# mic-rud/Learned-Compression-of-Point-Cloud-Geometry-and-Attributes

Hardware: AMD Instinct MI355X
Metric: encode+decode Mpoints/sec (higher is better)
Workload: dtype f32

## Files before the change

### include/pcc_hip.h

```cpp
#ifndef PCC_HIP_H
#define PCC_HIP_H

#include <stdint.h>

#ifdef __cplusplus
extern "C" {
#endif

#define PCC_OK 0
#define PCC_ERR_ARG (-1)
#define PCC_ERR_HIP (-2)
#define PCC_ERR_UNSUPPORTED (-3)
#define PCC_ERR_DATA (-4)

#define PCC_ACT_NONE 0
#define PCC_ACT_RELU 1
#define PCC_ACT_LEAKY_RELU 2

int pcc_version(void);
const char* pcc_last_error(void);
int pcc_device_count(void);
int pcc_device_name(int dev, char* out, int out_len);

int64_t pcc_hash_capacity(int64_t n);
// ... 24 lines not shown

int32_t pcc_color_jitter_chunk(void);
int64_t pcc_color_jitter_scratch_bytes(int64_t n, int32_t nbatch);
int pcc_color_jitter(const float* rgb, int64_t n, const int64_t* offsets, int32_t nbatch, const float* params,
                     const int32_t* order, float* out, void* scratch, int64_t scratch_bytes, void* stream);

int pcc_voxelize(const float* xyz, const int32_t* batch, int64_t n, int32_t nbatch, const float* attr, int32_t c,
                 float origin_x, float origin_y, float origin_z, float voxel, int32_t rounding, uint64_t* keys,
                 int32_t* vals, int64_t cap, int32_t* scratch, int32_t* out_coords, int32_t* out_first,
                 int32_t* out_npts, int64_t* out_sum, int32_t* out_row, int64_t* out_count, void* stream);

int pcc_kernel_map(const int32_t* out_coords, int64_t n_out, const uint64_t* in_keys,
                   const int32_t* in_vals, int64_t in_cap, int32_t ksize, int32_t step,
                   int32_t sign, int32_t* nbr, uint32_t* row_mask, int64_t* pair_count,
                   void* stream);

int pcc_pair_count(const uint32_t* row_mask, int64_t n_out, int64_t* pair_count, void* stream);

int64_t pcc_order_scratch_bytes(int64_t n);
int pcc_order_rows_by_mask(const uint32_t* row_mask, const int32_t* coords, int64_t n,
                           int32_t block_log2, int32_t tensor_stride, int32_t* order, uint32_t* group_mask32,
                           void* scratch, int64_t scratch_bytes, void* stream);
int pcc_permute_map_rows(const int32_t* nbr, const int32_t* order, int64_t n, int32_t K, int32_t* nbr_sorted, void* stream);

int64_t pcc_small_map_max(void);
int32_t pcc_small_paths(int32_t mask);
int pcc_small_kernel_map(const int32_t* out_coords, int64_t n_out, const uint64_t* in_keys, const int32_t* in_vals, int64_t in_cap,
                         int32_t ksize, int32_t step, int32_t sign, int32_t* nbr, uint32_t* row_mask, int32_t* order,
                         uint32_t* group_mask32, void* scratch, int64_t scratch_bytes, void* stream);

// ... 21 lines not shown
int pcc_epilogue_bwd(const float* dout, const float* c, const float* film, int64_t n, int32_t channels, int32_t act,
                     float* dc, float* dfilm, void* stream);

int64_t pcc_cast_colsum_scratch_elems(int32_t channels);
int pcc_cast_colsum(const float* x, int64_t n, int32_t channels, uint16_t* out_bf16, float* colsum, float* scratch,
                    int64_t scratch_elems, void* stream);

int64_t pcc_conv_packed_elems_x3(int32_t K, int32_t cin, int32_t cout);
int pcc_conv_pack_weights_x3(const float* w, int32_t K, int32_t cin, int32_t cout, uint16_t* w_packed, void* stream);
int pcc_conv_fwd_x3(const float* fin, int64_t n_in, int32_t cin, const uint16_t* w_packed, const float* bias,
                    const int32_t* nbr, const int32_t* order, const uint32_t* group_mask32, int32_t K, float* fout,
                    int64_t n_out, int32_t cout, int32_t act, const float* film, const float* residual, void* stream);

int pcc_im2col_thin(const float* fin, int32_t cin, const int32_t* nbr, int64_t n_out, int32_t K, float* out, int32_t k2,
                    void* stream);

int pcc_gather_sum_fwd(const float* scores, int32_t ld, const int32_t* nbr, int32_t K, int32_t cout,
                       const float* bias, float* out, int64_t n_out, int32_t act, void* stream);

int pcc_gather_rows(const float* src, int32_t c, const int32_t* idx, int64_t n, float* out,
                    int32_t accumulate, void* stream);

int pcc_scatter_rows(const float* src, int32_t c, const int32_t* idx, int64_t n, float* out,
                     void* stream);
int pcc_scatter_add_rows(const float* src, int32_t c, const int32_t* idx, int64_t n, float* out,
                         void* stream);

int pcc_compact_rows(const uint8_t* mask, int64_t n, const int32_t* coords, int32_t* out_coords,
                     const float* feats, int32_t c, float* out_feats, int32_t* new_index,
                     int32_t* scratch, int64_t* out_count, void* stream);
// ... 109 lines not shown
```

### learned-compression-of-point-cloud-geometry-and-attributes_amd/_lib.py

```python
import ctypes
import os
import subprocess

_HERE = os.path.dirname(os.path.abspath(__file__))
SO_PATH = os.path.join(_HERE, "libpcc_hip.so")
_lib = None

c_void_p, c_int, c_i32, c_i64 = ctypes.c_void_p, ctypes.c_int, ctypes.c_int32, ctypes.c_int64

SIGNATURES = {
    "pcc_version": (c_int, []),
    "pcc_last_error": (ctypes.c_char_p, []),
    "pcc_device_count": (c_int, []),
    "pcc_device_name": (c_int, [c_int, ctypes.c_char_p, c_int]),
    "pcc_hash_capacity": (c_i64, [c_i64]),
    "pcc_hash_build": (c_int, [c_void_p, c_i64, c_void_p, c_void_p, c_i64, c_i32, c_void_p, c_void_p]),
    "pcc_hash_lookup": (c_int, [c_void_p, c_void_p, c_i64, c_i32, c_void_p, c_i64, c_void_p, c_void_p]),
    "pcc_scan_scratch_elems": (c_i64, [c_i64]),
    "pcc_stride_map": (c_int, [c_void_p, c_i64, c_i32, c_void_p, c_void_p, c_i64, c_void_p, c_void_p, c_void_p, c_void_p]),
    "pcc_children": (c_int, [c_void_p, c_i64, c_i32, c_i32, c_void_p, c_void_p, c_i64, c_void_p, c_void_p, c_void_p, c_void_p]),
    "pcc_augment_rotate": (c_int, [c_void_p, c_i64, c_void_p, c_i32, ctypes.c_float, c_void_p, c_void_p, c_i64, c_void_p, c_void_p, c_void_p,
                                   c_void_p, c_void_p]),
    "pcc_color_jitter_chunk": (c_i32, []),
    "pcc_color_jitter_scratch_bytes": (c_i64, [c_i64, c_i32]),
    "pcc_color_jitter": (c_int, [c_void_p, c_i64, c_void_p, c_i32, c_void_p, c_void_p, c_void_p, c_void_p, c_i64, c_void_p]),
    "pcc_voxelize": (c_int, [c_void_p, c_void_p, c_i64, c_i32, c_void_p, c_i32, ctypes.c_float, ctypes.c_float, ctypes.c_float, ctypes.c_float,
                             c_i32, c_void_p, c_void_p, c_i64, c_void_p, c_void_p, c_void_p, c_void_p, c_void_p, c_void_p, c_void_p,
                             c_void_p]),
    "pcc_kernel_map": (c_int, [c_void_p, c_i64, c_void_p, c_void_p, c_i64, c_i32, c_i32, c_i32, c_void_p, c_void_p, c_void_p, c_void_p]),
    "pcc_pair_count": (c_int, [c_void_p, c_i64, c_void_p, c_void_p]),
    "pcc_conv_packed_elems": (c_i64, [c_i32, c_i32, c_i32]),
    "pcc_conv_pack_weights": (c_int, [c_void_p, c_i32, c_i32, c_i32, c_void_p, c_void_p]),
    "pcc_order_scratch_bytes": (c_i64, [c_i64]),
    "pcc_order_rows_by_mask": (c_int, [c_void_p, c_void_p, c_i64, c_i32, c_i32, c_void_p, c_void_p, c_void_p, c_i64, c_void_p]),
    "pcc_permute_map_rows": (c_int, [c_void_p, c_void_p, c_i64, c_i32, c_void_p, c_void_p]),
    "pcc_conv_fwd": (c_int, [c_void_p, c_i64, c_i32, c_void_p, c_void_p, c_void_p, c_void_p, c_void_p, c_void_p, c_i32,
                             c_void_p, c_i64, c_i32, c_i32, c_void_p, c_void_p, c_void_p]),
    "pcc_conv_small_max": (c_i64, [c_i64]),
    "pcc_conv_kernel_name": (c_int, [c_i32, c_i64, c_i32, c_i32, c_i64, c_i32, c_i32, ctypes.c_char_p, c_i32]),
    "pcc_small_map_max": (c_i64, []),
    "pcc_small_paths": (c_i32, [c_i32]),
    "pcc_small_kernel_map": (c_int, [c_void_p, c_i64, c_void_p, c_void_p, c_i64, c_i32, c_i32, c_i32, c_void_p, c_void_p, c_void_p,
                                     c_void_p, c_void_p, c_i64, c_void_p]),
    "pcc_conv_packed_elems_bf16": (c_i64, [c_i32, c_i32, c_i32]),
    "pcc_conv_pack_weights_bf16": (c_int, [c_void_p, c_i32, c_i32, c_i32, c_void_p, c_void_p]),
    "pcc_conv_fwd_bf16": (c_int, [c_void_p, c_i64, c_i32, c_void_p, c_void_p, c_void_p, c_void_p, c_void_p, c_i32, c_void_p, c_i64,
                                  c_i32, c_i32, c_void_p, c_void_p, c_void_p]),
    "pcc_conv_packed_elems_x3": (c_i64, [c_i32, c_i32, c_i32]),
    "pcc_conv_pack_weights_x3": (c_int, [c_void_p, c_i32, c_i32, c_i32, c_void_p, c_void_p]),
    "pcc_conv_fwd_x3": (c_int, [c_void_p, c_i64, c_i32, c_void_p, c_void_p, c_void_p, c_void_p, c_void_p, c_i32, c_void_p, c_i64,
                                c_i32, c_i32, c_void_p, c_void_p, c_void_p]),
    "pcc_epilogue_fwd": (c_int, [c_void_p, c_void_p, c_void_p, c_i64, c_i32, c_i32, c_void_p, c_void_p]),
    "pcc_cast_colsum_scratch_elems": (c_i64, [c_i32]),
    "pcc_cast_colsum": (c_int, [c_void_p, c_i64, c_i32, c_void_p, c_void_p, c_void_p, c_i64, c_void_p]),
    "pcc_epilogue_bwd": (c_int, [c_void_p, c_void_p, c_void_p, c_i64, c_i32, c_i32, c_void_p, c_void_p, c_void_p]),
    "pcc_im2col_thin": (c_int, [c_void_p, c_i32, c_void_p, c_i64, c_i32, c_void_p, c_i32, c_void_p]),
    "pcc_gather_sum_fwd": (c_int, [c_void_p, c_i32, c_void_p, c_i32, c_i32, c_void_p, c_void_p, c_i64, c_i32, c_void_p]),
    "pcc_gather_rows": (c_int, [c_void_p, c_i32, c_void_p, c_i64, c_void_p, c_i32, c_void_p]),
    "pcc_scatter_rows": (c_int, [c_void_p, c_i32, c_void_p, c_i64, c_void_p, c_void_p]),
    "pcc_scatter_add_rows": (c_int, [c_void_p, c_i32, c_void_p, c_i64, c_void_p, c_void_p]),
    "pcc_compact_rows": (c_int, [c_void_p, c_i64, c_void_p, c_void_p, c_void_p, c_i32, c_void_p, c_void_p, c_void_p, c_void_p, c_void_p]),
    "pcc_topk_state_elems": (c_i64, [c_i32]),
    "pcc_topk_mask": (c_int, [c_void_p, c_i32, c_void_p, c_i64, c_i32, c_void_p, c_void_p, c_void_p, c_void_p]),
    "pcc_count_per_batch": (c_int, [c_void_p, c_i64, c_i32, c_void_p, c_void_p]),
    "pcc_sort_scratch_bytes": (c_i64, [c_i64]),
    "pcc_sort_coords": (c_int, [c_void_p, c_i64, c_void_p, c_void_p, c_i64, c_void_p]),
    "pcc_kernel_map_transpose": (c_int, [c_void_p, c_i64, c_i32, c_i64, c_void_p, c_void_p, c_void_p]),
    "pcc_conv_wgrad_scratch_elems": (c_i64, [c_i32, c_i32, c_i32]),
    "pcc_conv_wgrad_kernel_name": (c_int, [c_i32, c_i32, c_i32, c_i32, c_i64, ctypes.c_char_p, c_i32, c_void_p, c_void_p]),
    "pcc_conv_wgrad": (c_int, [c_void_p, c_i64, c_i32, c_void_p, c_i64, c_i32, c_void_p, c_void_p, c_void_p, c_i32, c_void_p, c_void_p,
                               c_i64, c_void_p]),
    "pcc_conv_wgrad_bf16": (c_int, [c_void_p, c_i64, c_i32, c_void_p, c_i64, c_i32, c_void_p, c_void_p, c_void_p, c_i32, c_void_p, c_void_p,
# ... 40 lines not shown
def build(force=False):
    args = ["make", "-s", "-C", os.path.join(_HERE, "csrc"), "-j4"]
    if force:
        subprocess.check_call(args + ["clean"])
    subprocess.check_call(args)
    check_kernel_resources()
    check_kernel_resources(os.path.join(_HERE, "build", "rans_lanes.resources.txt"), LANE_KERNELS)
    check_kernel_resources(os.path.join(_HERE, "build", "chconv.resources.txt"), CHCONV_KERNELS)
    check_kernel_resources(os.path.join(_HERE, "build", "augment.resources.txt"), AUGMENT_KERNELS)
    check_kernel_resources(os.path.join(_HERE, "build", "normals.resources.txt"), NORMALS_KERNELS)
    check_kernel_resources(os.path.join(_HERE, "build", "voxelize.resources.txt"), VOXELIZE_KERNELS)
    check_small_kernel_lds_reads()
    return SO_PATH


NO_SCRATCH_KERNELS = ("conv_small_kernel", "conv_mfma_buf_kernel", "conv_mfma_kernel")
LANE_KERNELS = ("rans_lanes_encode_kernel", "rans_lanes_pack_kernel", "rans_lanes_decode_kernel")
CHCONV_KERNELS = ("chconv_kernel",)
AUGMENT_KERNELS = ("jitter_partial_kernel", "jitter_mean_kernel", "jitter_apply_kernel", "rotate_clear_kernel", "rotate_insert_kernel",
                   "rotate_flag_kernel", "rotate_finalize_kernel")

NORMALS_KERNELS = ("estimate_normals_kernel",)
VOXELIZE_KERNELS = ("voxelize_clear_kernel", "voxelize_insert_kernel", "voxelize_flag_kernel", "voxelize_finalize_kernel",
                    "voxelize_accumulate_kernel")


def check_small_kernel_lds_reads(obj=None):
    import glob
    import re
    import shutil
    objdump = "/opt/rocm/lib/llvm/bin/llvm-objdump"
# ... 141 lines not shown
```

### learned-compression-of-point-cloud-geometry-and-attributes_amd/blocks.py

```python
import os

import torch
import torch.nn as nn

from . import _threads
from . import sparse as sp
from .sparse import (ACT_NONE, ACT_RELU, ConvChain, CoordMap, MinkowskiConvolution,
                     MinkowskiGenerativeConvolutionTranspose, MinkowskiPruning, MinkowskiReLU, SparseTensor)


class _NonNegativeParametrizer(nn.Module):
    def __init__(self, minimum=0.0, reparam_offset=2 ** -18):
        super().__init__()
        pedestal = float(reparam_offset) ** 2
        self.register_buffer("pedestal", torch.tensor([pedestal]))
        self.lower_bound = _Bound((float(minimum) + pedestal) ** 0.5)


class _Bound(nn.Module):
    def __init__(self, bound):
        super().__init__()
        self.register_buffer("bound", torch.tensor([float(bound)]))


# ... 52 lines not shown
            with torch.cuda.stream(side):
                job(side)
        except BaseException as e:
            for h in handoffs:
                h.fail(e)
            raise

    if x_map.n >= PREFETCH_THREAD_MIN_ROWS:
        x_map._cache[("prefetch_job",)] = st.job_thread("pcc-map-prefetch", dev).submit(run)
    else:
        run()
    x_map._cache[done_key] = True
    return True


PREFETCH_THREAD_MIN_ROWS = 8192


def prefetch_up_maps(x_map):
    first = _threads.Handoff()

    def job(side):
        cand = x_map.up(3)
        x_map.mfma_kernel_map(cand, 3, True)
        first.set(side.record_event())
        cand.mfma_kernel_map(cand, 3)
        cand.kernel_map(cand, 3)
        x_map._cache[("prefetch_event",)] = side.record_event()

    if _start_prefetch(x_map, ("okmap_prefetched",), job, [first]):
# ... 81 lines not shown
            self.occ_predict = ConvChain(_conv(N_out, N_out), MinkowskiReLU(), _conv(N_out, N_out))

    def forward(self, x, coords=None, k=None, full_predictions=False):
        if not self.predict:
            return self._follow(x, coords)
        in_map = x.map
        _join_prefetch_first(in_map)
        x = self.conv(x)
        _join_prefetch(in_map)
        if self.dense and self.condition_ablation is None:
            x = self.conv_2(x)
        pred = self.occ_predict(x, last_out_channels=None if full_predictions else 1)
        nb = x.map._nbatch if x.map._nbatch is not None else x.map.nbatch
        mask = sp.topk_mask(pred.F, pred.C, k, nb)
        kept = min(max(int(k[0]), 0), x.map.n) if nb == 1 and len(k) == 1 and not torch.is_grad_enabled() else None
        coords_kept, feats_kept, _, _ = sp.compact_rows(mask, x.C, x.F, expected=kept)
        up_map = CoordMap(coords_kept, x.map.stride, nbatch=x.map._nbatch)
        x = SparseTensor(feats_kept, coordinate_map=up_map)
        if not self.dense and self.condition_ablation is None:
            x = self.conv_2(x)
        return x, pred, up_map

    def _follow(self, Q, up_map):
        if not isinstance(up_map, CoordMap):
            up_map = CoordMap(sp._as_int_coords(up_map), Q.map.stride // 2, nbatch=Q.map._nbatch)
        return self.conv(Q, out_map=up_map)


class ConditionEncoder(nn.Module):

    def __init__(self, C_in, N_scales, N_features, condition_ablation=None):
        super().__init__()
# ... 42 lines not shown
```

### learned-compression-of-point-cloud-geometry-and-attributes_amd/csrc/conv.hip

```cpp
#include <stdlib.h>

#include <type_traits>

#include "common.h"

namespace pcc {

typedef float f32x2 __attribute__((ext_vector_type(2)));
typedef float f32x4 __attribute__((ext_vector_type(4)));
typedef float f32x16 __attribute__((ext_vector_type(16)));
typedef __bf16 bf16x8 __attribute__((ext_vector_type(8)));

struct ConvArgs {
    const float* fin;
    const float* w;
    const float* wp;
    const float* bias;
    const int32_t* nbr;
    const int32_t* order;
    const uint32_t* gmask;
    float* fout;
    const float* film;
    const float* residual;
    int64_t n_in, n_out;
    int cin, cout, coutp, K, act;
    int bf16;
};

__device__ __forceinline__ float apply_act(float v, int act) {
    if (act == PCC_ACT_RELU) return v > 0.0f ? v : 0.0f;
    if (act == PCC_ACT_LEAKY_RELU) return v > 0.0f ? v : 0.01f * v;
    return v;
}

__global__ __launch_bounds__(256) void pack_weights_kernel(const float* __restrict__ w, int K, int cin, int cout,
                                                           int cinp, int coutp, float* __restrict__ wp) {
    const int64_t total = (int64_t)K * cinp * coutp;
    for (int64_t e = (int64_t)blockIdx.x * blockDim.x + threadIdx.x; e < total; e += (int64_t)gridDim.x * blockDim.x) {
        const int s = (int)(e & 3);
        int64_t t = e >> 2;
        const int col = (int)(t % coutp);
// ... 597 lines not shown
        }
    }

#pragma unroll
    for (int m = 0; m < MT; ++m) {
#pragma unroll
        for (int n = 0; n < NT; ++n) {
#pragma unroll
            for (int reg = 0; reg < 16; ++reg) {
                const int col = nt * BN + wcol + 32 * n + r;
                if (col >= a.cout) continue;
                const float bcol = a.bias ? a.bias[col] : 0.0f;
                const int64_t pos = row0 + wrow + 32 * m + (reg & 3) + 8 * (reg >> 2) + 4 * h;
                if (pos >= a.n_out) continue;
                const int64_t row = a.order ? a.order[pos] : pos;
                float v = acc[m][n][reg] + bcol;
                if (a.film) {
                    const float* fr = a.film + row * (2 * (int64_t)a.cout);
                    v = v * fr[col] + fr[a.cout + col];
                }
                v = apply_act(v, a.act);
                if (a.residual) v += a.residual[row * a.cout + col];
                a.fout[row * a.cout + col] = v;
            }
        }
    }
#endif
}

template <int SC, int NS>
// ... 492 lines not shown
static int launch_thin_cin(const ConvPlan& p, const ConvArgs& a, hipStream_t st) {
    switch (a.cin) {
        case 1: return launch_thin<1>(p, a, st);
        case 2: return launch_thin<2>(p, a, st);
        case 3: return launch_thin<3>(p, a, st);
        case 4: return launch_thin<4>(p, a, st);
        case 6: return launch_thin<6>(p, a, st);
        case 8: return launch_thin<8>(p, a, st);
        case 12: return launch_thin<12>(p, a, st);
        case 16: return launch_thin<16>(p, a, st);
        case 24: return launch_thin<24>(p, a, st);
        default: return PCC_ERR_UNSUPPORTED;
    }
}

static int conv_fwd(ConvMode mode, const ConvArgs& a, void* stream) {
    const char* who = CONV_ENTRY[mode];
    int rc = check_shape(a, mode, who);
    if (rc != PCC_OK) return rc;
    PCC_REQUIRE(a.act >= 0 && a.act <= 2, "%s: bad activation %d", who, a.act);
    if (mode == CONV_F32 && a.n_out <= 0) return PCC_OK;
    if (mode != CONV_F32 || a.cin % 32 == 0) {
        PCC_REQUIRE(a.wp != nullptr, "%s: MFMA path (cin=%d) needs packed weights", who, a.cin);
        PCC_REQUIRE(((reinterpret_cast<uintptr_t>(a.fin) | reinterpret_cast<uintptr_t>(a.wp)) & 15) == 0,
                    "%s: fin and w_packed must be 16-byte aligned (16-byte LDS-DMA loads)", who);
    } else {
        PCC_REQUIRE(a.w != nullptr, "%s: thin path (cin=%d) needs raw weights", who, a.cin);
    }
    if (a.n_out <= 0) return PCC_OK;
    ConvPlan p;
// ... 70 lines not shown
                    int32_t act, const float* film, const float* residual, void* stream) {
    return conv_fwd(CONV_X3, {fin, nullptr, reinterpret_cast<const float*>(w_packed), bias, nbr, order, group_mask32, fout, film,
                              residual, n_in, n_out, cin, cout, round_up32(cout), K, act, 0}, stream);
}

int pcc_im2col_thin(const float* fin, int32_t cin, const int32_t* nbr, int64_t n_out, int32_t K, float* out, int32_t k2,
                    void* stream) {
    PCC_REQUIRE(K >= 1 && K <= 27 && cin >= 1 && cin <= 16, "pcc_im2col_thin: bad shape (K=%d cin=%d)", K, cin);
    PCC_REQUIRE(k2 % 32 == 0 && k2 >= K * cin, "pcc_im2col_thin: row length %d must be a multiple of 32 and >= K * cin = %d", k2, K * cin);
    PCC_REQUIRE(nbr != nullptr && (reinterpret_cast<uintptr_t>(out) & 15) == 0, "pcc_im2col_thin: nbr required, out 16-byte aligned");
    if (n_out <= 0) return PCC_OK;
    hipLaunchKernelGGL(im2col_thin_kernel, dim3(blocks_for(n_out * (k2 / 4), 256, 1 << 20)), dim3(256), 0, as_stream(stream), fin, cin, nbr,
                       n_out, K, out, k2);
    PCC_LAUNCH_CHECK();
    return PCC_OK;
}

int pcc_gather_sum_fwd(const float* scores, int32_t ld, const int32_t* nbr, int32_t K, int32_t cout, const float* bias,
                       float* out, int64_t n_out, int32_t act, void* stream) {
    PCC_REQUIRE(K >= 1 && K <= 27 && cout >= 1 && ld >= K * cout, "pcc_gather_sum_fwd: bad shape (K=%d cout=%d ld=%d)", K, cout, ld);
    PCC_REQUIRE(nbr != nullptr, "pcc_gather_sum_fwd: neighbour table required");
    PCC_REQUIRE(act >= 0 && act <= 2, "pcc_gather_sum_fwd: bad activation %d", act);
    if (n_out <= 0) return PCC_OK;
    const unsigned nb27 = blocks_for(n_out, 256);
    const bool al16 = (reinterpret_cast<uintptr_t>(nbr) & 15) == 0;
#define PCC_GS27(C)                                                                                                    \
    hipLaunchKernelGGL(gather_sum27_kernel<C>, dim3(nb27), dim3(256), 0, as_stream(stream), scores, ld, nbr, bias, out, n_out, act)
    if (K == 27 && al16 && cout == 1) PCC_GS27(1);
    else if (K == 27 && al16 && cout == 2) PCC_GS27(2);
    else if (K == 27 && al16 && cout == 3) PCC_GS27(3);
// ... 45 lines not shown
```

### learned-compression-of-point-cloud-geometry-and-attributes_amd/csrc/coords.hip

```cpp
#include <stdarg.h>
#include <stdio.h>
#include <stdlib.h>

#include "common.h"
#include "sort.h"

namespace pcc {

static thread_local char g_err[512] = "";
void set_error(const char* fmt, ...) {
    va_list ap;
    va_start(ap, fmt);
    vsnprintf(g_err, sizeof(g_err), fmt, ap);
    va_end(ap);
}
const char* last_error() { return g_err; }

constexpr int SCAN_BLOCK = 256;
constexpr int SCAN_ITEMS = 4;
constexpr int SCAN_TILE = SCAN_BLOCK * SCAN_ITEMS;

__device__ __forceinline__ int wave_inclusive_scan(int v, int lane) {
#pragma unroll
    for (int d = 1; d < 64; d <<= 1) {
// ... 515 lines not shown
    if (threadIdx.x == 0 && pair_count && !row_mask && hits_s) atomicAdd(pair_count, (unsigned long long)hits_s);
}

__global__ __launch_bounds__(256) void pair_count_kernel(const uint32_t* __restrict__ row_mask, int64_t n,
                                                         unsigned long long* __restrict__ pair_count) {
    __shared__ unsigned long long ws[4];
    unsigned long long v = 0;
    for (int64_t i = (int64_t)blockIdx.x * 256 + threadIdx.x; i < n; i += (int64_t)gridDim.x * 256) v += __popc(row_mask[i]);
#pragma unroll
    for (int d = 32; d >= 1; d >>= 1) v += __shfl_xor(v, d, 64);
    if ((threadIdx.x & 63) == 0) ws[threadIdx.x >> 6] = v;
    __syncthreads();
    if (threadIdx.x == 0) {
        const unsigned long long t = ws[0] + ws[1] + ws[2] + ws[3];
        if (t) atomicAdd(pair_count, t);
    }
}

__global__ __launch_bounds__(256) void gather_rows_kernel(const float* __restrict__ src, int c,
                                                          const int32_t* __restrict__ idx, int64_t n,
                                                          float* __restrict__ out, int accumulate) {
    const int64_t total = n * c;
    for (int64_t e = (int64_t)blockIdx.x * blockDim.x + threadIdx.x; e < total; e += (int64_t)gridDim.x * blockDim.x) {
        const int64_t r = e / c;
        const int col = (int)(e - r * c);
        const int32_t s = idx[r];
        const float v = (s >= 0) ? src[(int64_t)s * c + col] : 0.0f;
        out[e] = accumulate ? out[e] + v : v;
    }
}
// ... 183 lines not shown
    if (ksize == 3) {
        if (pow2) hipLaunchKernelGGL(kernel_map27_kernel<true>, dim3(nb), dim3(256), 0, st, out_coords, n_out, in_keys, in_vals, tmask, tshift,
                                     sign * step, pitch, nbr, row_mask, pc);
        else hipLaunchKernelGGL(kernel_map27_kernel<false>, dim3(nb), dim3(256), 0, st, out_coords, n_out, in_keys, in_vals, tmask, tshift,
                                sign * step, pitch, nbr, row_mask, pc);
    } else {
        hipLaunchKernelGGL(kernel_map_kernel, dim3(nb), dim3(256), 0, st, out_coords, n_out, in_keys, in_vals, tmask, tshift, ksize, K,
                           sign * step, pitch, nbr, row_mask, pc);
    }
    if (pair_count && row_mask)
        hipLaunchKernelGGL(pair_count_kernel, dim3(blocks_for(n_out, 256 * 16, 512)), dim3(256), 0, st, row_mask, n_out, pc);
    PCC_LAUNCH_CHECK();
    return PCC_OK;
}

int pcc_pair_count(const uint32_t* row_mask, int64_t n_out, int64_t* pair_count, void* stream) {
    PCC_REQUIRE(pair_count != nullptr, "pcc_pair_count: no output");
    hipStream_t st = as_stream(stream);
    PCC_CHECK_HIP(hipMemsetAsync(pair_count, 0, sizeof(int64_t), st));
    if (n_out <= 0) return PCC_OK;
    hipLaunchKernelGGL(pair_count_kernel, dim3(blocks_for(n_out, 256 * 16, 512)), dim3(256), 0, st, row_mask, n_out,
                       reinterpret_cast<unsigned long long*>(pair_count));
    PCC_LAUNCH_CHECK();
    return PCC_OK;
}

int pcc_gather_rows(const float* src, int32_t c, const int32_t* idx, int64_t n, float* out, int32_t accumulate,
                    void* stream) {
    if (n <= 0 || c <= 0) return PCC_OK;
    hipLaunchKernelGGL(gather_rows_kernel, dim3(blocks_for(n * c, 256, 65536)), dim3(256), 0, as_stream(stream), src, c,
// ... 58 lines not shown
```

### learned-compression-of-point-cloud-geometry-and-attributes_amd/sparse.py

```python
import ctypes
import functools
import math
import weakref

import os

import torch
import torch.nn as nn

from . import _lib, _threads
from ._lib import check, ptr

ACT_NONE, ACT_RELU, ACT_LRELU = 0, 1, 2


def _require_cuda(t):
    if not t.is_cuda:
        raise RuntimeError("libpcc_hip operators need tensors on an MI355X device (got a CPU tensor); "
                           "there is no CPU fallback")


COORD_PROFILER = None


# ... 208 lines not shown
        if hit is not None:
            return hit
        keys, vals, cap = self.table()
        K = ksize ** 3
        n_out = out_map.n
        nbr = torch.empty((n_out, K), dtype=torch.int32, device=self.device)
        row_mask = torch.empty(n_out, dtype=torch.int32, device=self.device)
        step = self.stride // 2 if transposed else self.stride
        ev = _cp_begin()
        check(_lib.lib().pcc_kernel_map(ptr(out_map.coords), n_out, ptr(keys), ptr(vals), cap, ksize, step,
                                        -1 if transposed else 1, ptr(nbr), ptr(row_mask), None, _lib.stream()))
        pairs = PairCount(row_mask)
        probes = K * n_out if not transposed else max(n_out, K * n_out // 8)
        _cp_end(ev, "kernel_map", n_out, lambda: 20 * n_out + 8 * probes + 4 * int(pairs) + 4 * K * n_out)
        return self._keep_for(out_map, key, nbr, row_mask, pairs)

    def ordered_kernel_map(self, out_map, ksize, transposed=False):
        key = ("okmap", id(out_map), ksize, transposed, ORDER_BLOCK_LOG2)
        hit = self._cached_for(out_map, key)
        if hit is not None:
            return hit
        if (0 < out_map.n <= _small_map_max() and ksize in (2, 3) and ORDER_BLOCK_LOG2 < 0
                and ("kmap", id(out_map), ksize, transposed) not in self._cache):
            return self._small_ordered_kernel_map(out_map, ksize, transposed, key)
        nbr, row_mask, pairs = self.kernel_map(out_map, ksize, transposed)
        n_out = nbr.shape[0]
        ev = _cp_begin()
        order, gmask = _execution_order(row_mask, out_map.coords, n_out, out_map.stride)
        _cp_end(ev, "execution_order", n_out, 100 * n_out)
        return self._keep_for(out_map, key, nbr, order, gmask, pairs)
# ... 310 lines not shown
    if ev0 is not None:
        ev1 = torch.cuda.Event(enable_timing=True)
        ev1.record()
    PROFILER.append((name, cin, cout, pairs, n_out, ev0, ev1, gmask))


_MFMA_VISIT = (0, 4, 1, 5, 2, 6, 3, 7)


def _thin_im2col_forward(x_feats, in_map, out_map, layer, ksize, transposed, act, film, residual, out_channels):
    L = _lib.lib()
    w2p, bias, k2, cout = layer.im2col_weights(out_channels)
    nbr, _, pairs = in_map.kernel_map(out_map, ksize, transposed)
    n_out, K, cin = out_map.n, ksize ** 3, x_feats.shape[1]
    dev = x_feats.device
    x2 = torch.empty((n_out, k2), dtype=torch.float32, device=dev)
    out = torch.empty((n_out, cout), dtype=torch.float32, device=dev)
    ev0 = _prof_begin()
    ev = _cp_begin()
    check(L.pcc_im2col_thin(ptr(x_feats), cin, ptr(nbr), n_out, K, ptr(x2), k2, _lib.stream()))
    _cp_end(ev, "im2col_thin", n_out, lambda: 4 * K * n_out + 4 * cin * int(pairs) + 4 * k2 * n_out)
    check(L.pcc_conv_fwd(ptr(x2), n_out, k2, None, ptr(w2p), ptr(bias), None, None, None, 1, ptr(out), n_out, cout, act, ptr(film),
                         ptr(residual), _lib.stream()))
    _prof_end(ev0, f"thin_im2col<{cin}>", cin, cout, pairs, n_out)
    return out


def _narrow_head_forward(x_feats, in_map, out_map, layer, ksize, transposed, act, out_channels):
    L = _lib.lib()
    w_r, wp_r, bias, K, cout = layer.narrow_weights(out_channels)
    n_in, cin = x_feats.shape
    n_out = out_map.n
    nbr, _, pairs = in_map.kernel_map(out_map, ksize, transposed)
# ... 6 lines not shown
    ev = _cp_begin()
    check(L.pcc_gather_sum_fwd(ptr(scores), ld, ptr(nbr), K, cout, ptr(bias), ptr(out), n_out, act, _lib.stream()))
    _cp_end(ev, "gather_sum", n_out, lambda: 4 * K * n_out + 4 * cout * int(pairs) + 4 * cout * n_out)
    _prof_end(ev0, f"narrow_head<{cin}>", cin, cout, pairs, n_out)
    return out


def set_conv_small_max(workgroups):
    return int(_lib.lib().pcc_conv_small_max(int(workgroups)))


NARROW_HEAD_MAX_COUT = 4

CHECK_EXPECTED_COUNTS = os.environ.get("PCC_CHECK_COUNTS", "0") == "1"
ORDER_BLOCK_LOG2 = int(os.environ.get("PCC_ORDER_BLOCK_LOG2", "-1"))

INFER_BF16 = os.environ.get("PCC_INFER_BF16", "0") == "1"


def set_infer_bf16(enabled):
    global INFER_BF16
    INFER_BF16 = bool(enabled)


INFER_X3 = os.environ.get("PCC_INFER_X3", "0") == "1"


def set_infer_x3(enabled):
    global INFER_X3
    INFER_X3 = bool(enabled)
# ... 268 lines not shown
```

Before: 8.689.

## Fuse thin im2col gather into MFMA conv and derive kept-point kernel maps

Adds a conv kernel for thin-input layers that gathers neighbour features straight into LDS inside the MFMA GEMM. This drops the separate im2col pass and its intermediate buffer in global memory. It also adds a kernel that builds the self and transposed kernel maps for the kept points after top-k pruning by remapping the candidate maps through new_index, instead of redoing hash lookups. The gather path does per-element buffer loads, which may be less efficient than the old staged GEMM, and the derived maps depend on the cached candidate maps being present.

```diff
diff --git a/include/pcc_hip.h b/include/pcc_hip.h
--- a/include/pcc_hip.h
+++ b/include/pcc_hip.h
@@ -62,6 +62,10 @@
                    const int32_t* in_vals, int64_t in_cap, int32_t ksize, int32_t step,
                    int32_t sign, int32_t* nbr, uint32_t* row_mask, int64_t* pair_count,
                    void* stream);
+
+int pcc_kept_maps(const int32_t* new_index, int64_t n_cand, const int32_t* nbr_self_cand, const int32_t* nbr_t_cand,
+                  const uint32_t* mask_t_cand, int32_t* nbr_self_kept, uint32_t* mask_self_kept, int32_t* nbr_t_kept,
+                  uint32_t* mask_t_kept, void* stream);
 
 int pcc_pair_count(const uint32_t* row_mask, int64_t n_out, int64_t* pair_count, void* stream);
 
@@ -113,6 +117,10 @@
 
 int pcc_im2col_thin(const float* fin, int32_t cin, const int32_t* nbr, int64_t n_out, int32_t K, float* out, int32_t k2,
                     void* stream);
+
+int pcc_conv_fwd_thin_gather(const float* fin, int64_t n_in, int32_t cin, const float* w_packed, const float* bias,
+                             const int32_t* nbr, int32_t K, float* fout, int64_t n_out, int32_t cout, int32_t act,
+                             const float* film, const float* residual, void* stream);
 
 int pcc_gather_sum_fwd(const float* scores, int32_t ld, const int32_t* nbr, int32_t K, int32_t cout,
                        const float* bias, float* out, int64_t n_out, int32_t act, void* stream);
diff --git a/learned-compression-of-point-cloud-geometry-and-attributes_amd/_lib.py b/learned-compression-of-point-cloud-geometry-and-attributes_amd/_lib.py
--- a/learned-compression-of-point-cloud-geometry-and-attributes_amd/_lib.py
+++ b/learned-compression-of-point-cloud-geometry-and-attributes_amd/_lib.py
@@ -28,6 +28,7 @@
                              c_i32, c_void_p, c_void_p, c_i64, c_void_p, c_void_p, c_void_p, c_void_p, c_void_p, c_void_p, c_void_p,
                              c_void_p]),
     "pcc_kernel_map": (c_int, [c_void_p, c_i64, c_void_p, c_void_p, c_i64, c_i32, c_i32, c_i32, c_void_p, c_void_p, c_void_p, c_void_p]),
+    "pcc_kept_maps": (c_int, [c_void_p, c_i64, c_void_p, c_void_p, c_void_p, c_void_p, c_void_p, c_void_p, c_void_p, c_void_p]),
     "pcc_pair_count": (c_int, [c_void_p, c_i64, c_void_p, c_void_p]),
     "pcc_conv_packed_elems": (c_i64, [c_i32, c_i32, c_i32]),
     "pcc_conv_pack_weights": (c_int, [c_void_p, c_i32, c_i32, c_i32, c_void_p, c_void_p]),
@@ -55,7 +56,9 @@
     "pcc_cast_colsum": (c_int, [c_void_p, c_i64, c_i32, c_void_p, c_void_p, c_void_p, c_i64, c_void_p]),
     "pcc_epilogue_bwd": (c_int, [c_void_p, c_void_p, c_void_p, c_i64, c_i32, c_i32, c_void_p, c_void_p, c_void_p]),
     "pcc_im2col_thin": (c_int, [c_void_p, c_i32, c_void_p, c_i64, c_i32, c_void_p, c_i32, c_void_p]),
-    "pcc_gather_sum_fwd": (c_int, [c_void_p, c_i32, c_void_p, c_i32, c_i32, c_void_p, c_void_p, c_i64, c_i32, c_void_p]),
+    "pcc_conv_fwd_thin_gather": (c_int, [c_void_p, c_i64, c_i32, c_void_p, c_void_p, c_void_p, c_i32, c_void_p, c_i64, c_i32, c_i32, c_void_p,
+                                         c_void_p, c_void_p]),
+    "pcc_gather_sum_fwd":(c_int, [c_void_p, c_i32, c_void_p, c_i32, c_i32, c_void_p, c_void_p, c_i64, c_i32, c_void_p]),
     "pcc_gather_rows": (c_int, [c_void_p, c_i32, c_void_p, c_i64, c_void_p, c_i32, c_void_p]),
     "pcc_scatter_rows": (c_int, [c_void_p, c_i32, c_void_p, c_i64, c_void_p, c_void_p]),
     "pcc_scatter_add_rows": (c_int, [c_void_p, c_i32, c_void_p, c_i64, c_void_p, c_void_p]),
@@ -126,7 +129,7 @@
     return SO_PATH
 
 
-NO_SCRATCH_KERNELS = ("conv_small_kernel", "conv_mfma_buf_kernel", "conv_mfma_kernel")
+NO_SCRATCH_KERNELS = ("conv_small_kernel", "conv_mfma_buf_kernel", "conv_mfma_kernel", "conv_thin_gather_kernel")
 LANE_KERNELS = ("rans_lanes_encode_kernel", "rans_lanes_pack_kernel", "rans_lanes_decode_kernel")
 CHCONV_KERNELS = ("chconv_kernel",)
 AUGMENT_KERNELS = ("jitter_partial_kernel", "jitter_mean_kernel", "jitter_apply_kernel", "rotate_clear_kernel", "rotate_insert_kernel",
diff --git a/learned-compression-of-point-cloud-geometry-and-attributes_amd/blocks.py b/learned-compression-of-point-cloud-geometry-and-attributes_amd/blocks.py
--- a/learned-compression-of-point-cloud-geometry-and-attributes_amd/blocks.py
+++ b/learned-compression-of-point-cloud-geometry-and-attributes_amd/blocks.py
@@ -90,6 +90,7 @@
     return True
 
 
+DERIVE_KEPT_MAPS = os.environ.get("PCC_KEPT_MAPS", "1") != "0"
 PREFETCH_THREAD_MIN_ROWS = 8192
 
 
@@ -201,8 +202,11 @@
         nb = x.map._nbatch if x.map._nbatch is not None else x.map.nbatch
         mask = sp.topk_mask(pred.F, pred.C, k, nb)
         kept = min(max(int(k[0]), 0), x.map.n) if nb == 1 and len(k) == 1 and not torch.is_grad_enabled() else None
-        coords_kept, feats_kept, _, _ = sp.compact_rows(mask, x.C, x.F, expected=kept)
+        derive = DERIVE_KEPT_MAPS and not torch.is_grad_enabled()
+        coords_kept, feats_kept, new_index, n_kept = sp.compact_rows(mask, x.C, x.F, want_index=derive, expected=kept)
         up_map = CoordMap(coords_kept, x.map.stride, nbatch=x.map._nbatch)
+        if derive and n_kept > sp._small_map_max():
+            in_map.derive_kept_maps(x.map, new_index, up_map)
         x = SparseTensor(feats_kept, coordinate_map=up_map)
         if not self.dense and self.condition_ablation is None:
             x = self.conv_2(x)
diff --git a/learned-compression-of-point-cloud-geometry-and-attributes_amd/csrc/conv.hip b/learned-compression-of-point-cloud-geometry-and-attributes_amd/csrc/conv.hip
--- a/learned-compression-of-point-cloud-geometry-and-attributes_amd/csrc/conv.hip
+++ b/learned-compression-of-point-cloud-geometry-and-attributes_amd/csrc/conv.hip
@@ -25,6 +25,7 @@
     int64_t n_in, n_out;
     int cin, cout, coutp, K, act;
     int bf16;
+    int thin;
 };
 
 __device__ __forceinline__ float apply_act(float v, int act) {
@@ -652,6 +653,193 @@
                 const int64_t pos = row0 + wrow + 32 * m + (reg & 3) + 8 * (reg >> 2) + 4 * h;
                 if (pos >= a.n_out) continue;
                 const int64_t row = a.order ? a.order[pos] : pos;
+                float v = acc[m][n][reg] + bcol;
+                if (a.film) {
+                    const float* fr = a.film + row * (2 * (int64_t)a.cout);
+                    v = v * fr[col] + fr[a.cout + col];
+                }
+                v = apply_act(v, a.act);
+                if (a.residual) v += a.residual[row * a.cout + col];
+                a.fout[row * a.cout + col] = v;
+            }
+        }
+    }
+#endif
+}
+
+template <int BM, int BN>
+constexpr int conv_thin_gather_lds_bytes(int K) { return conv_lds_bytes<BM, BN>() + BM * K * (int)sizeof(int32_t); }
+
+template <int BM, int BN, int WAVES_M, int WAVES_N>
+__global__ __launch_bounds__(256) void conv_thin_gather_kernel(const ConvArgs a) {
+#if defined(__HIP_DEVICE_COMPILE__)
+    constexpr int RPT = BM / 32;
+    constexpr int WM = BM / WAVES_M, WN = BN / WAVES_N;
+    constexpr int MT = WM / 32, NT = WN / 32;
+    constexpr int A_ELEMS = BM * 32;
+    constexpr int W_ELEMS = 8 * BN * 4;
+    constexpr int W_LOADS = (8 * BN) / 256;
+    static_assert(WAVES_M * WAVES_N == 4 && MT >= 1 && MT <= 2 && NT >= 1 && W_LOADS >= 1, "bad tiling");
+
+    extern __shared__ __attribute__((aligned(16))) float smem[];
+    float* As = smem;
+    float* Ws = smem + 2 * A_ELEMS;
+    int32_t* idx_s = reinterpret_cast<int32_t*>(smem + 2 * A_ELEMS + 2 * W_ELEMS);
+
+    const int t = threadIdx.x;
+    const int lane = t & 63, wid = t >> 6;
+    const int r = lane & 31, h = lane >> 5;
+    const int wrow = (wid / WAVES_N) * WM, wcol = (wid % WAVES_N) * WN;
+
+    const int ntiles_n = a.coutp / BN;
+    const int64_t tile = blockIdx.x / ntiles_n;
+    const int nt = blockIdx.x - (int)(tile * ntiles_n);
+    const int64_t row0 = tile * BM;
+    const int K = a.K, thin = a.thin, kc = K * thin;
+    const int tshift = __builtin_ctz(thin);
+    const int cch = a.cin / 32;
+
+    {
+        const int64_t left = a.n_out - row0;
+        const int live = (int)(left < BM ? left : BM) * K;
+        const int32_t* src = a.nbr + row0 * K;
+        for (int e = t; e < BM * K; e += 256) idx_s[e] = (e < live) ? src[e] : -1;
+    }
+
+    __amdgpu_buffer_rsrc_t rsrc_a = __builtin_amdgcn_make_buffer_rsrc(
+        const_cast<float*>(a.fin), 0, (int)(uint32_t)(a.n_in * thin * 4), BUF_FLAGS);
+    __amdgpu_buffer_rsrc_t rsrc_w = __builtin_amdgcn_make_buffer_rsrc(
+        const_cast<float*>(a.wp), 0, (int)((uint32_t)a.cin * a.coutp * 4), BUF_FLAGS);
+
+    const int gchunk = t & 7;
+    int lbase[RPT], irow[RPT];
+    uint32_t a_dst[RPT];
+#pragma unroll
+    for (int i = 0; i < RPT; ++i) {
+        const int grow = wid * (BM / 4) + 8 * i + (lane >> 3);
+        const int q = gchunk ^ ((grow >> 1) & 7);
+        lbase[i] = 8 * (q >> 1) + (q & 1);
+        irow[i] = grow * K;
+        a_dst[i] = (uint32_t)(grow * 32 + gchunk * 4);
+    }
+    uint32_t w_voff[W_LOADS];
+#pragma unroll
+    for (int j = 0; j < W_LOADS; ++j) {
+        const int f = t + 256 * j;
+        const int g = f / BN, col = f - g * BN;
+        w_voff[j] = (uint32_t)((g * a.coutp + nt * BN + col) * 16);
+    }
+    const int wave_u = __builtin_amdgcn_readfirstlane(wid);
+    const uint32_t w_cstride = 8u * a.coutp * 16;
+    const uint32_t a_row_bytes = (uint32_t)thin * 4;
+
+    f32x4 gv[RPT];
+    auto gather = [&](int c) {
+#pragma unroll
+        for (int i = 0; i < RPT; ++i) {
+#pragma unroll
+            for (int s = 0; s < 4; ++s) {
+                const int logical = 32 * c + lbase[i] + 2 * s;
+                const bool col_ok = logical < kc;
+                const int k = col_ok ? (logical >> tshift) : 0;
+                const int ci = logical & (thin - 1);
+                const int idx = idx_s[irow[i] + k];
+                const uint32_t voff = (col_ok && idx >= 0) ? (uint32_t)idx * a_row_bytes + (uint32_t)ci * 4 : BUF_OOB;
+                gv[i][s] = __uint_as_float((uint32_t)__builtin_amdgcn_raw_buffer_load_b32(rsrc_a, voff, 0, 0));
+            }
+        }
+    };
+    auto store = [&](auto bufc) {
+        constexpr int buf = decltype(bufc)::value;
+#pragma unroll
+        for (int i = 0; i < RPT; ++i) *reinterpret_cast<f32x4*>(As + buf * A_ELEMS + a_dst[i]) = gv[i];
+    };
+    auto dma_w = [&](int c, auto bufc) {
+        constexpr int buf = decltype(bufc)::value;
+        const uint32_t wso = (uint32_t)c * w_cstride;
+#pragma unroll
+        for (int j = 0; j < W_LOADS; ++j)
+            __builtin_amdgcn_raw_ptr_buffer_load_lds(rsrc_w, (lds_ptr_t)(Ws + buf * W_ELEMS + (wave_u * 64 + 256 * j) * 4), 16,
+                                                     w_voff[j], wso, 0, 0);
+    };
+
+    const int sw = (r >> 1) & 7;
+    uint32_t a_addr[2][4], w_addr[2];
+#pragma unroll
+    for (int b = 0; b < 2; ++b) {
+#pragma unroll
+        for (int kk = 0; kk < 4; ++kk)
+            a_addr[b][kk] = (uint32_t)((b * A_ELEMS + (wrow + r) * 32 + (((kk ^ (sw >> 1)) << 1) | (h ^ (sw & 1))) * 4) * 4);
+        w_addr[b] = (uint32_t)((2 * A_ELEMS + b * W_ELEMS + (h * BN + wcol + r) * 4) * 4);
+    }
+    auto lds4 = [&](uint32_t addr) { return *reinterpret_cast<const f32x4*>(reinterpret_cast<const char*>(smem) + addr); };
+
+    f32x16 acc[MT][NT];
+#pragma unroll
+    for (int m = 0; m < MT; ++m)
+#pragma unroll
+        for (int n = 0; n < NT; ++n) {
+#pragma unroll
+            for (int i = 0; i < 16; ++i) acc[m][n][i] = 0.0f;
+        }
+
+    auto compute = [&](auto bufc) {
+        constexpr int buf = decltype(bufc)::value;
+        f32x4 av[2][MT], bv[2][NT];
+        __builtin_amdgcn_s_setprio(1);
+#pragma unroll
+        for (int m = 0; m < MT; ++m) av[0][m] = lds4(a_addr[buf][0] + 32 * m * 32 * 4);
+#pragma unroll
+        for (int n = 0; n < NT; ++n) bv[0][n] = lds4(w_addr[buf] + 32 * n * 16);
+#pragma unroll
+        for (int kk = 0; kk < 4; ++kk) {
+            const int cb = kk & 1, nb = cb ^ 1;
+            if (kk + 1 < 4) {
+#pragma unroll
+                for (int m = 0; m < MT; ++m) av[nb][m] = lds4(a_addr[buf][kk + 1] + 32 * m * 32 * 4);
+#pragma unroll
+                for (int n = 0; n < NT; ++n) bv[nb][n] = lds4(w_addr[buf] + (2 * (kk + 1) * BN + 32 * n) * 16);
+            }
+#pragma unroll
+            for (int s = 0; s < 4; ++s)
+#pragma unroll
+                for (int m = 0; m < MT; ++m)
+#pragma unroll
+                    for (int n = 0; n < NT; ++n)
+                        acc[m][n] = __builtin_amdgcn_mfma_f32_32x32x2f32(av[cb][m][s], bv[cb][n][s], acc[m][n], 0, 0, 0);
+        }
+        __builtin_amdgcn_s_setprio(0);
+    };
+
+    __syncthreads();
+    gather(0);
+    dma_w(0, std::integral_constant<int, 0>{});
+    store(std::integral_constant<int, 0>{});
+    __syncthreads();
+    auto step = [&](int c, auto bufc) {
+        constexpr int buf = decltype(bufc)::value;
+        gather(c + 1);
+        dma_w(c + 1, std::integral_constant<int, buf ^ 1>{});
+        compute(bufc);
+        store(std::integral_constant<int, buf ^ 1>{});
+        __syncthreads();
+    };
+    for (int c = 0; c < cch; c += 2) {
+        step(c, std::integral_constant<int, 0>{});
+        if (c + 1 < cch) step(c + 1, std::integral_constant<int, 1>{});
+    }
+
+#pragma unroll
+    for (int m = 0; m < MT; ++m) {
+#pragma unroll
+        for (int n = 0; n < NT; ++n) {
+#pragma unroll
+            for (int reg = 0; reg < 16; ++reg) {
+                const int col = nt * BN + wcol + 32 * n + r;
+                if (col >= a.cout) continue;
+                const float bcol = a.bias ? a.bias[col] : 0.0f;
+                const int64_t row = row0 + wrow + 32 * m + (reg & 3) + 8 * (reg >> 2) + 4 * h;
+                if (row >= a.n_out) continue;
                 float v = acc[m][n][reg] + bcol;
                 if (a.film) {
                     const float* fr = a.film + row * (2 * (int64_t)a.cout);
@@ -1174,6 +1362,43 @@
     }
 }
 
+template <int BM, int BN, int WM, int WN>
+static int launch_thin_gather(const ConvArgs& a, hipStream_t st) {
+    const int lds = conv_thin_gather_lds_bytes<BM, BN>(a.K);
+    return launch<conv_thin_gather_kernel<BM, BN, WM, WN>>((a.n_out + BM - 1) / BM * (a.coutp / BN), 256, lds,
+                                                            conv_thin_gather_lds_bytes<BM, BN>(27), a, st);
+}
+
+static int conv_fwd_thin_gather(const ConvArgs& a, void* stream) {
+    const char* who = "pcc_conv_fwd_thin_gather";
+    PCC_REQUIRE(a.K >= 1 && a.K <= 27, "%s: K=%d out of range", who, a.K);
+    PCC_REQUIRE(a.thin == 1 || a.thin == 2 || a.thin == 4 || a.thin == 8, "%s: cin must be 1, 2, 4 or 8 (got %d)", who, a.thin);
+    PCC_REQUIRE(a.K * a.thin <= 256, "%s: K * cin = %d exceeds 256", who, a.K * a.thin);
+    PCC_REQUIRE(a.cout >= 32 && a.cout % 32 == 0, "%s: cout must be a multiple of 32 (got %d)", who, a.cout);
+    PCC_REQUIRE(a.act >= 0 && a.act <= 2, "%s: bad activation %d", who, a.act);
+    PCC_REQUIRE(a.nbr != nullptr && a.fin != nullptr && a.wp != nullptr, "%s: fin, nbr and w_packed are required", who);
+    PCC_REQUIRE((reinterpret_cast<uintptr_t>(a.wp) & 15) == 0, "%s: w_packed must be 16-byte aligned (16-byte LDS-DMA loads)", who);
+    const uint64_t lim = BUF_OOB;
+    PCC_REQUIRE((uint64_t)a.n_in * a.thin * 4 <= lim && (uint64_t)a.n_out * a.K * 4 <= lim && (uint64_t)a.cin * a.coutp * 4 <= lim &&
+                    (uint64_t)a.n_out * a.cin * 4 <= lim,
+                "%s: operands of 4 GiB and more are not supported (use pcc_im2col_thin + pcc_conv_fwd)", who);
+    if (a.n_out <= 0) return PCC_OK;
+    ConvArgs gemm = a;
+    gemm.nbr = nullptr;
+    gemm.n_in = a.n_out;
+    gemm.K = 1;
+    ConvPlan p;
+    int rc = plan_conv(gemm, CONV_F32, p, who);
+    if (rc != PCC_OK) return rc;
+    hipStream_t st = as_stream(stream);
+    if (p.bm == 64 && p.bn == 64) return launch_thin_gather<64, 64, 2, 2>(a, st);
+    if (p.bm == 64 && p.bn == 128) return launch_thin_gather<64, 128, 2, 2>(a, st);
+    if (p.bm == 32) return launch_thin_gather<32, 128, 1, 4>(a, st);
+    if (p.bn == 64) return launch_thin_gather<128, 64, 2, 2>(a, st);
+    if (p.bn == 32) return launch_thin_gather<128, 32, 4, 1>(a, st);
+    return PCC_ERR_UNSUPPORTED;
+}
+
 static int conv_fwd(ConvMode mode, const ConvArgs& a, void* stream) {
     const char* who = CONV_ENTRY[mode];
     int rc = check_shape(a, mode, who);
@@ -1274,6 +1499,15 @@
                        n_out, K, out, k2);
     PCC_LAUNCH_CHECK();
     return PCC_OK;
+}
+
+int pcc_conv_fwd_thin_gather(const float* fin, int64_t n_in, int32_t cin, const float* w_packed, const float* bias, const int32_t* nbr,
+                             int32_t K, float* fout, int64_t n_out, int32_t cout, int32_t act, const float* film, const float* residual,
+                             void* stream) {
+    ConvArgs a = {};
+    a.fin = fin; a.wp = w_packed; a.bias = bias; a.nbr = nbr; a.fout = fout; a.film = film; a.residual = residual;
+    a.n_in = n_in; a.n_out = n_out; a.thin = cin; a.cin = round_up32(K * cin); a.cout = cout; a.coutp = round_up32(cout); a.K = K; a.act = act;
+    return conv_fwd_thin_gather(a, stream);
 }
 
 int pcc_gather_sum_fwd(const float* scores, int32_t ld, const int32_t* nbr, int32_t K, int32_t cout, const float* bias,
diff --git a/learned-compression-of-point-cloud-geometry-and-attributes_amd/csrc/coords.hip b/learned-compression-of-point-cloud-geometry-and-attributes_amd/csrc/coords.hip
--- a/learned-compression-of-point-cloud-geometry-and-attributes_amd/csrc/coords.hip
+++ b/learned-compression-of-point-cloud-geometry-and-attributes_amd/csrc/coords.hip
@@ -553,6 +553,51 @@
     if (threadIdx.x == 0) {
         const unsigned long long t = ws[0] + ws[1] + ws[2] + ws[3];
         if (t) atomicAdd(pair_count, t);
+    }
+}
+
+__global__ __launch_bounds__(256) void kept_maps_kernel(const int32_t* __restrict__ new_index, int64_t n_cand,
+                                                        const int32_t* __restrict__ nbr_self_cand,
+                                                        const int32_t* __restrict__ nbr_t_cand,
+                                                        const uint32_t* __restrict__ mask_t_cand,
+                                                        int32_t* __restrict__ nbr_self_kept, uint32_t* __restrict__ mask_self_kept,
+                                                        int32_t* __restrict__ nbr_t_kept, uint32_t* __restrict__ mask_t_kept) {
+    __shared__ int32_t ni[64];
+    __shared__ unsigned rm[64];
+    __shared__ int any_s;
+    const int64_t row0 = (int64_t)blockIdx.x * 64;
+    const int nrows = (int)((n_cand - row0 < 64) ? (n_cand - row0) : 64);
+    if (threadIdx.x == 0) any_s = 0;
+    __syncthreads();
+    if (threadIdx.x < 64) {
+        const int32_t v = ((int)threadIdx.x < nrows) ? new_index[row0 + threadIdx.x] : -1;
+        ni[threadIdx.x] = v;
+        rm[threadIdx.x] = 0u;
+        if (v >= 0) any_s = 1;
+    }
+    __syncthreads();
+    if (!any_s) return;
+    const int total = nrows * 27;
+    for (int e = threadIdx.x; e < total; e += 256) {
+        const int lr = e / 27, k = e - lr * 27;
+        const int32_t dst = ni[lr];
+        if (dst < 0) continue;
+        const int64_t src_e = row0 * 27 + e, dst_e = (int64_t)dst * 27 + k;
+        if (nbr_self_cand) {
+            const int32_t j = nbr_self_cand[src_e];
+            const int32_t v = (j >= 0) ? new_index[j] : -1;
+            nbr_self_kept[dst_e] = v;
+            if (v >= 0) atomicOr(&rm[lr], 1u << k);
+        }
+        if (nbr_t_cand) nbr_t_kept[dst_e] = nbr_t_cand[src_e];
+    }
+    __syncthreads();
+    if ((int)threadIdx.x < nrows) {
+        const int32_t dst = ni[threadIdx.x];
+        if (dst >= 0) {
+            if (nbr_self_cand) mask_self_kept[dst] = rm[threadIdx.x];
+            if (nbr_t_cand) mask_t_kept[dst] = mask_t_cand[row0 + threadIdx.x];
+        }
     }
 }
 
@@ -766,6 +811,20 @@
     return PCC_OK;
 }
 
+int pcc_kept_maps(const int32_t* new_index, int64_t n_cand, const int32_t* nbr_self_cand, const int32_t* nbr_t_cand,
+                  const uint32_t* mask_t_cand, int32_t* nbr_self_kept, uint32_t* mask_self_kept, int32_t* nbr_t_kept,
+                  uint32_t* mask_t_kept, void* stream) {
+    PCC_REQUIRE(n_cand < (1ll << 31), "pcc_kept_maps: too many rows");
+    PCC_REQUIRE(new_index != nullptr || n_cand <= 0, "pcc_kept_maps: new_index required");
+    PCC_REQUIRE(!nbr_self_cand || (nbr_self_kept && mask_self_kept), "pcc_kept_maps: self map asked for without its outputs");
+    PCC_REQUIRE(!nbr_t_cand || (mask_t_cand && nbr_t_kept && mask_t_kept), "pcc_kept_maps: second map asked for without its mask or outputs");
+    if (n_cand <= 0 || (!nbr_self_cand && !nbr_t_cand)) return PCC_OK;
+    hipLaunchKernelGGL(kept_maps_kernel, dim3(blocks_for(n_cand, 64)), dim3(256), 0, as_stream(stream), new_index, n_cand, nbr_self_cand,
+                       nbr_t_cand, mask_t_cand, nbr_self_kept, mask_self_kept, nbr_t_kept, mask_t_kept);
+    PCC_LAUNCH_CHECK();
+    return PCC_OK;
+}
+
 int pcc_pair_count(const uint32_t* row_mask, int64_t n_out, int64_t* pair_count, void* stream) {
     PCC_REQUIRE(pair_count != nullptr, "pcc_pair_count: no output");
     hipStream_t st = as_stream(stream);
diff --git a/learned-compression-of-point-cloud-geometry-and-attributes_amd/sparse.py b/learned-compression-of-point-cloud-geometry-and-attributes_amd/sparse.py
--- a/learned-compression-of-point-cloud-geometry-and-attributes_amd/sparse.py
+++ b/learned-compression-of-point-cloud-geometry-and-attributes_amd/sparse.py
@@ -246,6 +246,24 @@
         probes = K * n_out if not transposed else max(n_out, K * n_out // 8)
         _cp_end(ev, "kernel_map", n_out, lambda: 20 * n_out + 8 * probes + 4 * int(pairs) + 4 * K * n_out)
         return self._keep_for(out_map, key, nbr, row_mask, pairs)
+
+    def derive_kept_maps(self, cand, new_index, kept_map):
+        k_self, k_t = ("kmap", id(cand), 3, False), ("kmap", id(cand), 3, True)
+        hit_self, hit_t = cand._cached_for(cand, k_self), self._cached_for(cand, k_t)
+        if hit_self is None or hit_t is None or hit_self[0].shape[1] != 27 or hit_t[0].shape[1] != 27:
+            return False
+        n, dev = kept_map.n, self.device
+        nbr_s = torch.empty((n, 27), dtype=torch.int32, device=dev)
+        nbr_t = torch.empty((n, 27), dtype=torch.int32, device=dev)
+        mask_s = torch.empty(n, dtype=torch.int32, device=dev)
+        mask_t = torch.empty(n, dtype=torch.int32, device=dev)
+        ev = _cp_begin()
+        check(_lib.lib().pcc_kept_maps(ptr(new_index), cand.n, ptr(hit_self[0]), ptr(hit_t[0]), ptr(hit_t[1]), ptr(nbr_s), ptr(mask_s),
+                                       ptr(nbr_t), ptr(mask_t), _lib.stream()))
+        _cp_end(ev, "kept_maps", n, 4 * cand.n + (4 * 27 * 5 + 12) * n)
+        kept_map._keep_for(kept_map, ("kmap", id(kept_map), 3, False), nbr_s, mask_s, PairCount(mask_s))
+        self._keep_for(kept_map, ("kmap", id(kept_map), 3, True), nbr_t, mask_t, PairCount(mask_t))
+        return True
 
     def ordered_kernel_map(self, out_map, ksize, transposed=False):
         key = ("okmap", id(out_map), ksize, transposed, ORDER_BLOCK_LOG2)
@@ -586,9 +604,14 @@
     nbr, _, pairs = in_map.kernel_map(out_map, ksize, transposed)
     n_out, K, cin = out_map.n, ksize ** 3, x_feats.shape[1]
     dev = x_feats.device
-    x2 = torch.empty((n_out, k2), dtype=torch.float32, device=dev)
     out = torch.empty((n_out, cout), dtype=torch.float32, device=dev)
     ev0 = _prof_begin()
+    if THIN_GATHER and max(x_feats.shape[0] * cin, n_out * K, k2 * cout) * 4 < 0xFFFFF000:
+        check(L.pcc_conv_fwd_thin_gather(ptr(x_feats), x_feats.shape[0], cin, ptr(w2p), ptr(bias), ptr(nbr), K, ptr(out), n_out, cout,
+                                         act, ptr(film), ptr(residual), _lib.stream()))
+        _prof_end(ev0, f"thin_im2col<{cin}>", cin, cout, pairs, n_out)
+        return out
+    x2 = torch.empty((n_out, k2), dtype=torch.float32, device=dev)
     ev = _cp_begin()
     check(L.pcc_im2col_thin(ptr(x_feats), cin, ptr(nbr), n_out, K, ptr(x2), k2, _lib.stream()))
     _cp_end(ev, "im2col_thin", n_out, lambda: 4 * K * n_out + 4 * cin * int(pairs) + 4 * k2 * n_out)
@@ -625,6 +648,7 @@
 
 CHECK_EXPECTED_COUNTS = os.environ.get("PCC_CHECK_COUNTS", "0") == "1"
 ORDER_BLOCK_LOG2 = int(os.environ.get("PCC_ORDER_BLOCK_LOG2", "-1"))
+THIN_GATHER = os.environ.get("PCC_THIN_GATHER", "1") != "0"
 
 INFER_BF16 = os.environ.get("PCC_INFER_BF16", "0") == "1"
 
```

After: 8.722 (median of 6 runs). No clear change (+0.4%).
